# nizepart/Research-and-Development-of-Kubernetes-Operator-for-Machine-Learning-Pipelines

Hardware: AMD Instinct MI355X
Metric: served_tokens_per_sec (higher is better)
Workload: dtype bf16

## Files before the change

### research-and-development-of-kubernetes-operator-for-machine-learning-pipelines_amd/ops/csrc/bindings.cpp

```cpp
#include <cstdlib>
#include <string>
#include <torch/library.h>
#include <ATen/ATen.h>
#include <c10/hip/HIPStream.h>
#include <c10/core/DeviceGuard.h>
#include <cmath>

#include "launch.h"
#include "gemm_plan.h"

namespace {

using at::Tensor;

hipStream_t cur_stream() { return c10::hip::getCurrentHIPStream().stream(); }

void check_bf16(const Tensor& t, const char* name) {
  TORCH_CHECK(t.is_cuda(), name, " must be a GPU tensor");
  TORCH_CHECK(t.scalar_type() == at::kBFloat16, name, " must be bf16");
  TORCH_CHECK(t.is_contiguous(), name, " must be contiguous");
}
void check_i32(const Tensor& t, const char* name) {
  TORCH_CHECK(t.is_cuda(), name, " must be a GPU tensor");
  TORCH_CHECK(t.scalar_type() == at::kInt, name, " must be int32");
// ... 898 lines not shown
  const long H = mlop::ep_hidden((long)h), k = mlop::ep_topk((long)h);
  check_bf16(out, "out"); check_bf16(y, "y"); check_i32(topi, "topi");
  TORCH_CHECK(topw.scalar_type() == at::kFloat && topw.is_cuda() && topw.is_contiguous(), "topw fp32");
  TORCH_CHECK(out.dim() == 2 && out.size(1) == H && y.dim() == 2 && y.size(1) == H, "ep_combine: [*, H] rows");
  TORCH_CHECK(topw.numel() == out.size(0) * k && topi.numel() == out.size(0) * k, "ep_combine: [T, k] routing");
  c10::DeviceGuard g(out.device());
  mlop::ep_combine((long)h, out.data_ptr(), y.data_ptr(), (long)y.size(0), topw.data_ptr<float>(),
                   topi.data_ptr<int>(), (int)out.size(0), cur_stream());
}
int64_t ep_error(int64_t h) { return mlop::ep_error((long)h); }
int64_t ep_mem_mode(int64_t h) { return mlop::ep_mem_mode((long)h); }
void ep_destroy(int64_t h) { mlop::ep_destroy((long)h); }

}

extern "C" const char* mlop_src_hash();
std::string src_hash() { return std::string(mlop_src_hash()); }

TORCH_LIBRARY(mlop, m) {
  m.def("src_hash() -> str", &src_hash);
  m.def("device_delay(int us) -> ()", &device_delay);
  m.def("car_create(int rank, int world, int max_bytes, int device, bool split=False) -> int", &car_create);
  m.def("car_ipc_handle(int h) -> Tensor", &car_ipc_handle);
  m.def("car_open(int h, Tensor handles) -> ()", &car_open);
  m.def("car_all_reduce(int h, Tensor(a!) out, Tensor inp, bool two_shot=False) -> ()");
  m.def("car_all_reduce_add(int h, Tensor(a!) residual, Tensor inp) -> ()");
  m.def("car_broadcast(int h, Tensor(a!) buf, int root) -> ()");
  m.def("car_all_gather(int h, Tensor(a!) out, Tensor piece) -> ()");
  m.def("car_error(int h) -> int", &car_error);
  m.def("attn_fused_max_pairs(int n) -> int", &attn_fused_max_pairs);
  m.def("car_mem_mode(int h) -> int", &car_mem_mode);
  m.def("car_destroy(int h) -> ()", &car_destroy);
  m.def("chan_create(str name, int slots, int consumers) -> int", &chan_create);
  m.def("chan_open(str name) -> int", &chan_open);
  m.def("chan_send(int h, Tensor vals, int timeout_us) -> bool", &chan_send);
  m.def("chan_recv(int h, int consumer, Tensor(a!) out, int timeout_us) -> bool", &chan_recv);
  m.def("chan_unlink(str name) -> ()", &chan_unlink);
  m.def("chan_close(int h, bool unlink) -> ()", &chan_close);
  m.def("xg_create(str name, int world, int slots, int max_words) -> int", &xg_create);
  m.def("xg_open(str name, int rank) -> int", &xg_open);
  m.def("xg_exchange(int h, Tensor vals, Tensor(a!) out, Tensor(b!) counts, int timeout_us) -> bool", &xg_exchange);
  m.def("xg_close(int h) -> ()", &xg_close);
  m.def("ep_create(int rank, int world, int E, int k, int H, int tcap, int device) -> int", &ep_create);
  m.def("ep_ipc_handle(int h) -> Tensor", &ep_ipc_handle);
  m.def("ep_open(int h, Tensor handles) -> ()", &ep_open);
  m.def("ep_dispatch(int h, Tensor(a!) xp, Tensor(b!) offsets, Tensor x, Tensor topi) -> ()");
  m.def("ep_combine(int h, Tensor(a!) out, Tensor y, Tensor topw, Tensor topi) -> ()");
  m.def("ep_error(int h) -> int", &ep_error);
  m.def("ep_mem_mode(int h) -> int", &ep_mem_mode);
  m.def("ep_destroy(int h) -> ()", &ep_destroy);
  m.def("gemm_workspace(int M, int N, int K, int epi) -> int", &gemm_workspace);
  m.def("gemm_big_variant(int set=-1) -> int", &knob<mlop::gemm_big_variant>);
  m.def("gemm_half_tile(int set=-1) -> int", &knob<mlop::gemm_half_tile>);
  m.def("gemm_small_nt(int set=-1) -> int", &knob<mlop::gemm_small_nt>);
  m.def("attn_kv_nt(int set=-1) -> int", &knob<mlop::attn_kv_nt>);
  m.def("gemm_slab_nt(int set=-1) -> int", &knob<mlop::gemm_slab_nt>);
  m.def("gemm_rope_split(int set=-1) -> int", &knob<mlop::gemm_rope_split>);
  m.def("gemm_split_target(int set=-1) -> int", &knob<mlop::gemm_split_target>);
  m.def("gemm_grouped_narrow(int set=-1) -> int", &knob<mlop::gemm_grouped_narrow>);
  m.def("gemm_ws_max_m(int set=-1) -> int", &knob<mlop::gemm_ws_max_m>);
  m.def("decode_chain_max_m() -> int", &decode_chain_max_m);
  m.def("gemm_ws_plan(int rb, int u, int nt) -> ()", &gemm_ws_plan);
  m.def("gemm_ws_small_m(int set=-1) -> int", &knob<mlop::gemm_ws_small_m>);
  m.def("gemm_ws_rope_m(int set=-1) -> int", &knob<mlop::gemm_ws_rope_m>);
  m.def("flash_persist(int set=-1) -> int", &knob<mlop::flash_persist>);
  m.def("flash_stream(int set=-1) -> int", &knob<mlop::flash_stream>);
  m.def("gemm_grouped_balance(int set=-1) -> int", &knob<mlop::gemm_grouped_balance>);
  m.def("gemm_grouped_order(int set=-1) -> int", &knob<mlop::gemm_grouped_order>);
  m.def("moe_mid_tok(int set=-1) -> int", &knob<mlop::moe_mid_tok>);
  m.def("gemm_mid_chain(int set=-1) -> int", &knob<mlop::gemm_mid_chain>);
  m.def("mid_chain_ok(int M, int N, int K, int epi) -> bool", &mid_chain_ok);
  m.def("moe_mid_max_tokens(int set=-1) -> int", &knob<mlop::moe_mid_max_tokens>);
  m.def("gemm_grouped_plan(int bm, int bn, int stages, int splits) -> ()", &gemm_grouped_plan);
  m.def("gemm_dense_plan(int variant, int bm, int bn, int splits, int stages=0) -> ()", &gemm_dense_plan);
  m.def("gemm_small_stages(int set=-1) -> int", &knob<mlop::gemm_small_stages>);
  m.def("gemm_small_tile(int set=-1) -> int", &knob<mlop::gemm_small_tile>);
  m.def("gemm_sk_mode(int set=-1) -> int", &knob<mlop::gemm_sk_mode>);
  m.def("gemm_sk_reserve() -> bool", &gemm_sk_reserve);
  m.def("gemm_sk_workgroups(int M, int N, int K) -> int", &gemm_sk_workgroups);
  m.def("vmm_supported(int device) -> bool", &vmm_supported);
  m.def("vmm_granularity(int device) -> int", &vmm_granularity);
  m.def("vmm_arena(int bytes, int device) -> Tensor", &vmm_arena);
  m.def("vmm_map_chunks(Tensor flat, int region_stride, int n_regions, int chunk_bytes, int first, "
        "int count, bool async_) -> bool", &vmm_map_chunks);
  m.def("vmm_chunks_ready(Tensor flat) -> int", &vmm_chunks_ready);
  m.def("vmm_error(Tensor flat) -> int", &vmm_error);
  m.def("gemm_rope_supported(int M, int N, int K) -> bool", &gemm_rope_supported);
  m.def("w4_chain_ok(int M, int N, int K) -> bool", &w4_chain_ok);
  m.def("chain_ok(int M, int N, int K, int epi) -> bool", &chain_ok);
  m.def("gemm_route(int M, int N, int K, int op, int n_groups=0, int rows_per_group=0) -> int[]", &gemm_route);
  m.def("gemm_route_env(int M, int N, int K, int op, int cus, bool sk, int n_groups=0, int rows_per_group=0) -> int[]", &gemm_route_env);
  m.def("gemm_tile_configs() -> int[]", &gemm_tile_configs);
  m.def("gemm_res_ss(Tensor(a!) residual, Tensor a, Tensor w, Tensor(b!) ss_out) -> bool");
  m.def("gemm_rs(Tensor(a!) out, Tensor a, Tensor w, Tensor ss_in, float eps, int epi) -> bool");
  m.def("gemm_rs_rope(Tensor(a!) q_out, Tensor(b!) k_cache, Tensor(c!) v_cache, Tensor a, Tensor w, "
        "Tensor pos, Tensor cos_sin, Tensor slots, Tensor ss_in, float eps) -> bool");
  m.def("gemm_rope_cache(Tensor(a!) q_out, Tensor(b!) k_cache, Tensor(c!) v_cache, Tensor a, Tensor w, "
        "Tensor pos, Tensor cos_sin, Tensor slots) -> bool");
  m.def("gemm(Tensor(a!) out, Tensor a, Tensor w, Tensor(b!) ws, int epi) -> ()");
  m.def("grouped_gemm(Tensor(a!) out, Tensor a, Tensor w, Tensor offsets, int max_rows, "
        "int epi, Tensor? a_rows=None) -> ()");
  m.def("gemm_add_rmsnorm(Tensor(a!) out, Tensor(b!) residual, Tensor a, Tensor w, Tensor norm_w, "
        "Tensor(c!) ws, float eps) -> bool");
  m.def("gemv_chain_supported(int M, int N, int K, int epi) -> bool", &gemv_chain_supported);
  m.def("moe_route(Tensor(a!) topw, Tensor(b!) topi, Tensor logits) -> ()");
  m.def("moe_permute(Tensor(a!) xp, Tensor(b!) offsets, Tensor(c!) src, Tensor(d!) inv, Tensor x, "
// ... 86 lines not shown
```

### research-and-development-of-kubernetes-operator-for-machine-learning-pipelines_amd/ops/csrc/gemm_plan.cc

```cpp
#include "gemm_plan.h"

#include <algorithm>
#include <stddef.h>
#include <stdexcept>

namespace mlop {

namespace {
enum { EPI_NONE = 0, EPI_SILU_MUL = 1, EPI_ROPE = 3 };
enum { WS_NONE = 0, WS_SILU_MUL = 1, WS_ROPE = 3, WS_RES = 5 };
constexpr int kHeadD = 128;
constexpr int kGroupedSmallStages = 3;
}

static PlanEnv g_knobs;
PlanEnv& gemm_knobs() { return g_knobs; }

int gemm_split_target(int set) {
  if (set >= 1) g_knobs.split_target = set;
  return g_knobs.split_target;
}

int gemm_small_stages(int set) {
  if (set >= 0) g_knobs.small_stages = set;
  return g_knobs.small_stages;
}

int gemm_small_tile(int set) {
  if (set >= 0) g_knobs.small_tile = set;
  return g_knobs.small_tile;
}

static bool tile_shape_built(int bm, int bn, bool grouped) {
  for (const TileCfg& t : kGemmTiles)
    if (t.BM == bm && t.BN == bn && (grouped || !(bm == 256 && bn == 256))) return true;
  return false;
}

void gemm_grouped_plan(int bm, int bn, int stages, int splits) {
  if (bm > 0 && !tile_shape_built(bm, bn, true))
    throw std::runtime_error("gemm_grouped_plan: no grouped config for this tile");
  int* gp = g_knobs.gp;
  gp[0] = bm, gp[1] = bn, gp[2] = stages, gp[3] = splits;
}

void gemm_dense_plan(int variant, int bm, int bn, int splits, int stages) {
  if (variant >= 0 && variant != 0 && variant != 1 && variant != 3 && variant != 5 && variant != 6)
    throw std::runtime_error("gemm_dense_plan: variant must be 0, 1, 3, 5 or 6");
  if (variant == 0 && !tile_shape_built(bm, bn, false))
    throw std::runtime_error("gemm_dense_plan: no dense config for this tile");
  int* dp = g_knobs.dp;
  dp[0] = variant, dp[1] = bm, dp[2] = bn, dp[3] = splits, dp[4] = stages > 0 ? stages : 0;
}

int gemm_big_variant(int set) {
  if (set >= 0) g_knobs.big_variant = set;
  return g_knobs.big_variant;
}
int gemm_grouped_narrow(int set) {
  if (set >= 0) g_knobs.grouped_narrow = set;
  return g_knobs.grouped_narrow;
}
int gemm_half_tile(int set) {
  if (set >= 0) g_knobs.half_tile = set;
  return g_knobs.half_tile;
}

int gemm_sk_mode(int set) {
  if (set >= 0) g_knobs.sk_mode = set;
  return g_knobs.sk_mode;
}

int gemm_rope_split(int set) {
  if (set >= 1) g_knobs.rope_split_k = set;
  return g_knobs.rope_split_k;
}

int gemm_mid_chain(int set) {
  if (set >= 0) g_knobs.mid_chain = set;
  return g_knobs.mid_chain;
}

int gemm_ws_max_m(int set) {
  if (set >= 0) g_knobs.ws_max_m = set > 64 ? 64 : set;
  return g_knobs.ws_max_m;
}

int gemm_ws_small_m(int set) {
  if (set >= 0) g_knobs.ws_small_m = set > 64 ? 64 : set;
  return g_knobs.ws_small_m;
}

int gemm_ws_rope_m(int set) {
  if (set >= 0) g_knobs.ws_rope_m = set > 64 ? 64 : set;
  return g_knobs.ws_rope_m;
}


bool gemv_takes(const PlanEnv& e, int M, int N, int K, int epi) {
  if (M < 1 || M > e.gemv_max_m || K % 8 || N < 4) return false;
  if (epi == EPI_SILU_MUL) return N % 32 == 0;
  if (epi == EPI_ROPE) return N % kHeadD == 0;
  return epi == EPI_NONE && N % 4 == 0;
}

bool gemv_grouped_takes(int M, int N, int K, int epi) {
  return M >= 1 && M <= 8 && K % 8 == 0 && N % (epi == EPI_SILU_MUL ? 32 : 4) == 0 &&
         (epi == EPI_NONE || epi == EPI_SILU_MUL);
}

bool gemv_chain_takes(const PlanEnv& e, int M, int N, int K, int epi) {
  return M <= e.gemv_chain_max_m && gemv_takes(e, M, N, K, epi);
}

bool ws_prefer(const PlanEnv& e, int M, int N, int K, int epi) {
  if (M <= e.gemv_chain_max_m || (long)N * K > 32L * 1024 * 1024 || K % 512) return false;
  if (epi == WS_ROPE) return M <= e.ws_rope_m && N % 128 == 0;
  return M <= e.ws_small_m && (epi == WS_NONE || epi == WS_RES) && N % 16 == 0;
// ... 407 lines not shown
```

### research-and-development-of-kubernetes-operator-for-machine-learning-pipelines_amd/ops/csrc/gemm_plan.h

```cpp
#pragma once

#if defined(__HIP__) || defined(__HIPCC__)
#define MLOP_HD __host__ __device__
#else
#define MLOP_HD
#endif

namespace mlop {

constexpr int kBK = 64;
constexpr int kMaxSplits = 8;
constexpr int kSkMaxWg = 256;
constexpr long kSkScratchFloats = 2l * kSkMaxWg * 256 * 256;
constexpr int kSkMinIters = 16;
constexpr int sk_min_half() { return kSkMinIters / 2 > 1 ? kSkMinIters / 2 : 1; }

MLOP_HD inline int sk_choose_d(int T, int nk, int cus, int min_half) {
  const int r = T % cus;
  if (r == 0) return 0;
  float best = 0.9f * nk;
  int best_d = 0;
  const int dmax = cus / r < 32 ? cus / r : 32;
  for (int d = 2; d <= dmax; ++d) {
    if (nk % d || nk / d < min_half) continue;
    const float w = 0.04f * r * d;
    const float cost = nk / d + (w > 2.f ? w : 2.f) + 2.f * (d >= 3 ? d : d - 1) + 1.f;
    if (cost < best) {
      best = cost;
      best_d = d;
    }
  }
  return best_d;
}

struct PlanEnv {
  int cus = 0;
  bool sk = false;
  int small_tile = 1;
  int small_stages = 3;
  int big_variant = 5;
  int half_tile = 1;
  int grouped_narrow = 1;
  int split_target = 512;
  int rope_split_k = 2;
  int sk_mode = 1;
  int mid_chain = 0;
  int gp[4] = {-1, -1, -1, -1};
  int dp[5] = {-1, -1, -1, -1, 0};
  int ws_small_m = 8, ws_rope_m = 8, ws_max_m = 0;
  int gemv_max_m = 4, gemv_chain_max_m = 4;
  bool sk_on() const { return sk_mode && sk && cus > 0; }
};
PlanEnv& gemm_knobs();
PlanEnv gemm_live_env();
int gemm_small_tile(int set);
int gemm_small_stages(int set);
int gemm_big_variant(int set);
int gemm_half_tile(int set);
int gemm_grouped_narrow(int set);
int gemm_split_target(int set);
int gemm_rope_split(int set);
int gemm_sk_mode(int set);
int gemm_mid_chain(int set);
int gemm_ws_small_m(int set);
int gemm_ws_rope_m(int set);
int gemm_ws_max_m(int set);

enum GemmOp {
  OP_PLAIN = 0,
  OP_SILU_MUL = 1,
  OP_ADD_RMSNORM = 2,
  OP_ROPE = 3,
  OP_CHAIN_RES_SS = 4,
  OP_CHAIN_RS = 8,
  OP_CHAIN_RS_SILU = 9,
  OP_CHAIN_RS_ROPE = 11,
  OP_GROUPED = 16,
  OP_GROUPED_SILU = 17,
};

struct GemmCall {
  int op = OP_PLAIN;
  int M = 0, N = 0, K = 0;
  int lda = 0, ldb = 0, ldc = 0;
  int n_groups = 0, rows_per_group = 0;
  long ws_avail = -1;
  bool indirect = false;
};

enum GemmFamily { FAM_REFUSED = 0, FAM_GEMV, FAM_WS, FAM_TILE, FAM_PP, FAM_W4, FAM_W4H };
enum GemmFinish { FIN_NONE = 0, FIN_REDUCE, FIN_ADD_RMSNORM, FIN_ROPE_SLABS, FIN_RMSNORM };
enum GemmWsSrc { WS_SRC_NONE = 0, WS_SRC_CALLER, WS_SRC_SCRATCH };

#define MLOP_GEMM_TILES(X)       \
  X(16, 32, 1, 2, 8, false, 0)   \
  X(16, 32, 1, 2, 6, false, 0)   \
  X(16, 32, 1, 2, 4, false, 0)   \
  X(16, 64, 1, 2, 8, false, 0)   \
  X(16, 64, 1, 2, 6, false, 0)   \
  X(16, 64, 1, 2, 4, false, 0)   \
  X(32, 32, 1, 2, 8, false, 0)   \
  X(32, 32, 1, 2, 4, false, 0)   \
  X(32, 64, 1, 4, 6, false, 0)   \
  X(32, 64, 1, 4, 4, false, 0)   \
  X(64, 32, 1, 2, 4, false, 0)   \
  X(64, 64, 1, 4, 6, false, 0)   \
  X(64, 64, 1, 4, 4, false, 0)   \
  X(64, 64, 1, 4, 3, false, 0)   \
  X(128, 64, 2, 2, 5, false, 0)  \
  X(128, 64, 2, 2, 3, false, 0)  \
  X(256, 64, 4, 2, 3, false, 0)  \
// ... 52 lines not shown
```

### research-and-development-of-kubernetes-operator-for-machine-learning-pipelines_amd/ops/csrc/gemm_w4.hip

```cpp
#include "common.h"
#include "launch.h"
#include "gemm_plan.h"
#include "gemm_w4_asm.h"

#include <type_traits>
#include <utility>

namespace mlop {

namespace {
enum { W4_NONE = 0, W4_SILU_MUL = 1, W4_ROPE = 3, W4_ADD_SS = 4, W4_RS = 8 };
using i32x4 = __attribute__((ext_vector_type(4))) int;
typedef __attribute__((address_space(3))) uint16_t lds_u16;

__device__ __forceinline__ i32x4 make_srd(const void* p) {
  const uint64_t a = (uint64_t)p;
  i32x4 r;
  r.x = __builtin_amdgcn_readfirstlane((int)(uint32_t)a);
  r.y = __builtin_amdgcn_readfirstlane((int)(uint32_t)(a >> 32));
  r.z = 0x7fffffff;
  r.w = 0x00020000;
  return r;
}

template <int I>
__device__ __forceinline__ void read_block(float (&v)[32]) {
#define MLOP_W4_OUTS                                                                                   \
  "=v"(v[0]), "=v"(v[1]), "=v"(v[2]), "=v"(v[3]), "=v"(v[4]), "=v"(v[5]), "=v"(v[6]), "=v"(v[7]),     \
      "=v"(v[8]), "=v"(v[9]), "=v"(v[10]), "=v"(v[11]), "=v"(v[12]), "=v"(v[13]), "=v"(v[14]),         \
      "=v"(v[15]), "=v"(v[16]), "=v"(v[17]), "=v"(v[18]), "=v"(v[19]), "=v"(v[20]), "=v"(v[21]),       \
      "=v"(v[22]), "=v"(v[23]), "=v"(v[24]), "=v"(v[25]), "=v"(v[26]), "=v"(v[27]), "=v"(v[28]),       \
      "=v"(v[29]), "=v"(v[30]), "=v"(v[31])
  if constexpr (I == 0) asm volatile(MLOP_W4_READ0_ASM : MLOP_W4_OUTS);
  else if constexpr (I == 1) asm volatile(MLOP_W4_READ1_ASM : MLOP_W4_OUTS);
  else if constexpr (I == 2) asm volatile(MLOP_W4_READ2_ASM : MLOP_W4_OUTS);
  else if constexpr (I == 3) asm volatile(MLOP_W4_READ3_ASM : MLOP_W4_OUTS);
  else if constexpr (I == 4) asm volatile(MLOP_W4_READ4_ASM : MLOP_W4_OUTS);
  else if constexpr (I == 5) asm volatile(MLOP_W4_READ5_ASM : MLOP_W4_OUTS);
  else if constexpr (I == 6) asm volatile(MLOP_W4_READ6_ASM : MLOP_W4_OUTS);
  else asm volatile(MLOP_W4_READ7_ASM : MLOP_W4_OUTS);
#undef MLOP_W4_OUTS
}

template <typename F, int... I>
__device__ __forceinline__ void unroll_impl(F& f, std::integer_sequence<int, I...>) {
  (f(std::integral_constant<int, I>{}), ...);
}
template <int N, typename F>
__device__ __forceinline__ void unroll(F&& f) {
  unroll_impl(f, std::make_integer_sequence<int, N>{});
}
}

template <int EPI, int BMT>
__global__ void __launch_bounds__(256, 1) gemm_w4_kernel(
    const uint16_t* __restrict__ A, int lda, const uint16_t* __restrict__ B, int ldb,
    uint16_t* __restrict__ C, int ldc, int M, int N, int K, int n_tiles_x, int m_tiles, int group_m,
    RopeEpi re, int n_dp, int n_items, float* __restrict__ ws, int* __restrict__ cnt) {
  constexpr int BM = BMT, BN = 256;
  static_assert(BMT == 256 || BMT == 128, "tile heights of the generated K-loops");
  constexpr int NI = BMT / 32;
  constexpr int NPC = NI + 8;
  constexpr int BASE = EPI & 3;
  constexpr bool ADD = (EPI & W4_ADD_SS) != 0, RS = (EPI & W4_RS) != 0;
  static_assert(!ADD || BASE == W4_NONE, "residual add on the plain epilogue only");
  constexpr int NS = BASE == W4_SILU_MUL ? 2 * NI : 4 * NI;
  extern __shared__ __attribute__((aligned(16))) uint16_t smem[];
  const int tid = threadIdx.x, lane = tid & 63;
  const int wid = __builtin_amdgcn_readfirstlane(tid >> 6);
  const int wm = wid >> 1, wn = wid & 1;
  const int nk = K / 64;

  const int G = gridDim.x, Lb = blockIdx.x;
  const int q = G >> 3, rr = G & 7, xcd = Lb & 7, slot = Lb >> 3;
  const int lid = (xcd < rr ? xcd * (q + 1) : rr * (q + 1) + (xcd - rr) * q) + slot;
  auto origin = [&](int t, int& m0, int& n0) {
    const int band = t / (group_m * n_tiles_x), in_band = t % (group_m * n_tiles_x);
    const int gm_here = min(group_m, m_tiles - band * group_m);
    m0 = (band * group_m + in_band % gm_here) * BM;
    n0 = (in_band / gm_here) * BN;
    if constexpr (BASE == W4_ROPE) n0 = (n_tiles_x - 1) * BN - n0;
  };
  auto item = [&](int i, int& m0, int& n0, int& kb, int& nkl) {
    const bool tail = i >= n_dp;
    origin(tail ? n_dp + ((i - n_dp) >> 1) : i, m0, n0);
    kb = tail ? ((i - n_dp) & 1) * (nk >> 1) : 0;
    nkl = tail ? nk >> 1 : nk;
  };
  auto dma_offsets = [&](int m0, int n0, int kb, uint32_t (&vo)[NPC]) {
#pragma unroll
    for (int i = 0; i < NPC; ++i) {
      const int p = wid + 4 * i;
      const int r = (i < NI ? p : p - 4 * NI) * 8 + (lane >> 3);
      const uint32_t ch = (uint32_t)(((lane & 7) ^ ((r >> 1) & 7)) << 4);
      if (i < NI) vo[i] = (uint32_t)min(m0 + r, M - 1) * (uint32_t)(lda * 2) + ch + kb * 128;
      else vo[i] = (uint32_t)min(n0 + r, N - 1) * (uint32_t)(ldb * 2) + ch + kb * 128;
    }
  };
  const i32x4 srdA = make_srd(A), srdB = make_srd(B);
  const auto srdC = __builtin_amdgcn_make_buffer_rsrc((void*)C, 0, (int)((uint32_t)M * (uint32_t)ldc * 2u), 0x00020000);
  const uint32_t lbase = (uint32_t)(uintptr_t)((lds_u16*)smem);
  const uint32_t sw = ((lane & 15) >> 1) & 7;
  const uint32_t c0 = (((uint32_t)(lane >> 4)) ^ sw) << 4, c1 = (((uint32_t)(lane >> 4) + 4) ^ sw) << 4;
  const uint32_t a_row = lbase + (uint32_t)(wm * (BMT / 2) + (lane & 15)) * 128;
  const uint32_t b_row = lbase + BMT * 128 + (uint32_t)(wn * 128 + (lane & 15)) * 128;
  const uint32_t dbase0 = __builtin_amdgcn_readfirstlane(lbase + wid * 1024);
  const uint32_t k128 = 128;
  float* rinv_lds = reinterpret_cast<float*>(smem + 65536);
  int* band_flag = reinterpret_cast<int*>(smem + 65536 + 1024);

  for (int it = lid, first = 1; it < n_items; it += G, first = 0) {
    int m0, n0, kb, nkl;
    item(it, m0, n0, kb, nkl);
    uint32_t vo[NPC], vn[NPC];
    dma_offsets(m0, n0, kb, vo);
    const bool next = it + G < n_items;
    {
      int m1 = m0, n1 = n0, kb1 = kb, nkl1 = nkl;
      if (next) item(it + G, m1, n1, kb1, nkl1);
      dma_offsets(m1, n1, kb1, vn);
    }
    if constexpr (RS) {
      const auto rs_ss = __builtin_amdgcn_make_buffer_rsrc((void*)re.ss_in, 0, (int)((uint32_t)M * 4u), 0x00020000);
      const uint32_t voff = (uint32_t)(m0 + wm * (BMT / 2) + lane) * 4u;
      const uint32_t lds_dst = __builtin_amdgcn_readfirstlane(lbase + 131072u + (uint32_t)wid * 512u);
      uint32_t msave;
      asm volatile(
          "s_mov_b32 %[ms], m0\n"
          "s_mov_b32 m0, %[dst]\n"
          "s_nop 0\n"
          "buffer_load_dword %[vo], %[srd], 0 offen lds\n"
          "s_add_u32 m0, m0, 0x100\n"
          "s_nop 0\n"
          "buffer_load_dword %[vo2], %[srd], 0 offen lds\n"
          "s_mov_b32 m0, %[ms]\n"
          : [ms] "=&s"(msave)
          : [dst] "s"(lds_dst), [vo] "v"(voff), [vo2] "v"(voff + 256u), [srd] "s"(rs_ss)
          : "memory", "scc");
    }
    uint32_t rA0 = a_row + c0, rA1 = a_row + c1, rB0 = b_row + c0, rB1 = b_row + c1;
    uint32_t dbase = dbase0, koff = 256, m0save;
    uint32_t iter = __builtin_amdgcn_readfirstlane(nkl - 3);
    const uint32_t s_first = __builtin_amdgcn_readfirstlane(first), s_next = __builtin_amdgcn_readfirstlane((int)next);
    bf16x8 fa0_0, fa0_1, fa0_2, fa0_3, fa0_4, fa0_5, fa0_6, fa0_7;
    bf16x8 fb0_0, fb0_1, fb0_2, fb0_3, fb0_4, fb0_5, fb0_6, fb0_7;
    bf16x8 fa1_0, fa1_1, fa1_2, fa1_3, fa1_4, fa1_5, fa1_6, fa1_7;
    bf16x8 fb1_0, fb1_1, fb1_2, fb1_3, fb1_4, fb1_5, fb1_6, fb1_7;
#define MLOP_W4_OPERANDS                                                                                         \
  : [fa0_0] "=&v"(fa0_0), [fa0_1] "=&v"(fa0_1), [fa0_2] "=&v"(fa0_2), [fa0_3] "=&v"(fa0_3),                      \
    [fa0_4] "=&v"(fa0_4), [fa0_5] "=&v"(fa0_5), [fa0_6] "=&v"(fa0_6), [fa0_7] "=&v"(fa0_7),                      \
    [fb0_0] "=&v"(fb0_0), [fb0_1] "=&v"(fb0_1), [fb0_2] "=&v"(fb0_2), [fb0_3] "=&v"(fb0_3),                      \
    [fb0_4] "=&v"(fb0_4), [fb0_5] "=&v"(fb0_5), [fb0_6] "=&v"(fb0_6), [fb0_7] "=&v"(fb0_7),                      \
    [fa1_0] "=&v"(fa1_0), [fa1_1] "=&v"(fa1_1), [fa1_2] "=&v"(fa1_2), [fa1_3] "=&v"(fa1_3),                      \
    [fa1_4] "=&v"(fa1_4), [fa1_5] "=&v"(fa1_5), [fa1_6] "=&v"(fa1_6), [fa1_7] "=&v"(fa1_7),                      \
    [fb1_0] "=&v"(fb1_0), [fb1_1] "=&v"(fb1_1), [fb1_2] "=&v"(fb1_2), [fb1_3] "=&v"(fb1_3),                      \
    [fb1_4] "=&v"(fb1_4), [fb1_5] "=&v"(fb1_5), [fb1_6] "=&v"(fb1_6), [fb1_7] "=&v"(fb1_7),                      \
    [rA0] "+v"(rA0), [rA1] "+v"(rA1), [rB0] "+v"(rB0), [rB1] "+v"(rB1), [koff] "+s"(koff), [dbase] "+s"(dbase), \
    [iter] "+s"(iter), [m0save] "=&s"(m0save)                                                                    \
  : [vo0] "v"(vo[0]), [vo1] "v"(vo[1]), [vo2] "v"(vo[2]), [vo3] "v"(vo[3]), [vo4] "v"(vo[4]), [vo5] "v"(vo[5]), \
    [vo6] "v"(vo[6]), [vo7] "v"(vo[7]), [vo8] "v"(vo[8]), [vo9] "v"(vo[9]), [vo10] "v"(vo[10]),                 \
    [vo11] "v"(vo[11]), [vo12] "v"(vo[12]), [vo13] "v"(vo[13]), [vo14] "v"(vo[14]), [vo15] "v"(vo[15]),         \
    [vn0] "v"(vn[0]), [vn1] "v"(vn[1]), [vn2] "v"(vn[2]), [vn3] "v"(vn[3]), [vn4] "v"(vn[4]), [vn5] "v"(vn[5]), \
    [vn6] "v"(vn[6]), [vn7] "v"(vn[7]), [vn8] "v"(vn[8]), [vn9] "v"(vn[9]), [vn10] "v"(vn[10]),                 \
    [vn11] "v"(vn[11]), [vn12] "v"(vn[12]), [vn13] "v"(vn[13]), [vn14] "v"(vn[14]), [vn15] "v"(vn[15]),         \
    [srdA] "s"(srdA), [srdB] "s"(srdB), [k128] "s"(k128), [first] "s"(s_first), [has_next] "s"(s_next)          \
  : "memory", "scc", MLOP_W4_AGPR_CLOBBERS
#define MLOP_W4H_OPERANDS                                                                                        \
  : [fa0_0] "=&v"(fa0_0), [fa0_1] "=&v"(fa0_1), [fa0_2] "=&v"(fa0_2), [fa0_3] "=&v"(fa0_3),                      \
    [fb0_0] "=&v"(fb0_0), [fb0_1] "=&v"(fb0_1), [fb0_2] "=&v"(fb0_2), [fb0_3] "=&v"(fb0_3),                      \
    [fb0_4] "=&v"(fb0_4), [fb0_5] "=&v"(fb0_5), [fb0_6] "=&v"(fb0_6), [fb0_7] "=&v"(fb0_7),                      \
    [fa1_0] "=&v"(fa1_0), [fa1_1] "=&v"(fa1_1), [fa1_2] "=&v"(fa1_2), [fa1_3] "=&v"(fa1_3),                      \
    [fb1_0] "=&v"(fb1_0), [fb1_1] "=&v"(fb1_1), [fb1_2] "=&v"(fb1_2), [fb1_3] "=&v"(fb1_3),                      \
    [fb1_4] "=&v"(fb1_4), [fb1_5] "=&v"(fb1_5), [fb1_6] "=&v"(fb1_6), [fb1_7] "=&v"(fb1_7),                      \
    [rA0] "+v"(rA0), [rA1] "+v"(rA1), [rB0] "+v"(rB0), [rB1] "+v"(rB1), [koff] "+s"(koff), [dbase] "+s"(dbase), \
    [iter] "+s"(iter), [m0save] "=&s"(m0save)                                                                    \
  : [vo0] "v"(vo[0]), [vo1] "v"(vo[1]), [vo2] "v"(vo[2]), [vo3] "v"(vo[3]), [vo4] "v"(vo[4]), [vo5] "v"(vo[5]), \
    [vo6] "v"(vo[6]), [vo7] "v"(vo[7]), [vo8] "v"(vo[8]), [vo9] "v"(vo[9]), [vo10] "v"(vo[10]),                 \
    [vo11] "v"(vo[11]), [vn0] "v"(vn[0]), [vn1] "v"(vn[1]), [vn2] "v"(vn[2]), [vn3] "v"(vn[3]),                 \
    [vn4] "v"(vn[4]), [vn5] "v"(vn[5]), [vn6] "v"(vn[6]), [vn7] "v"(vn[7]), [vn8] "v"(vn[8]), [vn9] "v"(vn[9]), \
    [vn10] "v"(vn[10]), [vn11] "v"(vn[11]), [srdA] "s"(srdA), [srdB] "s"(srdB), [k128] "s"(k128),               \
    [first] "s"(s_first), [has_next] "s"(s_next)                                                                 \
  : "memory", "scc", MLOP_W4_AGPR_CLOBBERS
    constexpr int NQ = NS + (RS ? 2 : 0);
    if constexpr (BMT == 256) {
      static_assert(NQ == 32 || NQ == 16 || NQ == 34 || NQ == 18, "one generated K-loop per VMEM count");
      if constexpr (NQ == 32) asm volatile(MLOP_W4_KLOOP_S32_P0_ASM MLOP_W4_OPERANDS);
      else if constexpr (NQ == 16) asm volatile(MLOP_W4_KLOOP_S16_P0_ASM MLOP_W4_OPERANDS);
      else if constexpr (NQ == 34) asm volatile(MLOP_W4_KLOOP_S34_P0_ASM MLOP_W4_OPERANDS);
      else asm volatile(MLOP_W4_KLOOP_S18_P0_ASM MLOP_W4_OPERANDS);
    } else {
      static_assert(NQ == 16 || NQ == 8 || NQ == 18 || NQ == 10, "one generated K-loop per VMEM count");
      if constexpr (NQ == 16) asm volatile(MLOP_W4H_KLOOP_S16_ASM MLOP_W4H_OPERANDS);
      else if constexpr (NQ == 8) asm volatile(MLOP_W4H_KLOOP_S8_ASM MLOP_W4H_OPERANDS);
      else if constexpr (NQ == 18) asm volatile(MLOP_W4H_KLOOP_S18_ASM MLOP_W4H_OPERANDS);
      else asm volatile(MLOP_W4H_KLOOP_S10_ASM MLOP_W4H_OPERANDS);
    }
#undef MLOP_W4_OPERANDS
#undef MLOP_W4H_OPERANDS

    const int lr = wm * (BMT / 2) + (lane & 15), qd = lane >> 4;
    const bool part = it >= n_dp;
    const int sidx = part ? it - n_dp : 0;
    const auto rs_other = __builtin_amdgcn_make_buffer_rsrc(part ? ws + (size_t)(sidx ^ 1) * 65536 : (float*)C, 0,
                                                           65536 * 4, 0x00020000);
    if (part) {
      const int tt = sidx >> 1;
      const auto rs_own = __builtin_amdgcn_make_buffer_rsrc(ws + (size_t)sidx * 65536, 0, 65536 * 4, 0x00020000);
      auto put = [&](auto I_) {
        constexpr int I = decltype(I_)::value;
        float v[32];
        read_block<I>(v);
#pragma unroll
        for (int q4 = 0; q4 < 8; ++q4)
          __builtin_amdgcn_raw_buffer_store_b128(
              u32x4{__float_as_uint(v[4 * q4]), __float_as_uint(v[4 * q4 + 1]), __float_as_uint(v[4 * q4 + 2]),
                    __float_as_uint(v[4 * q4 + 3])},
              rs_own, (uint32_t)(((I * 8 + q4) * 256 + tid) * 16), 0, 16 );
      };
      unroll<NI>(put);
      asm volatile("s_waitcnt vmcnt(0)" ::: "memory");
      __syncthreads();
      int* flag = reinterpret_cast<int*>(smem);
      if (tid == 0) {
        const int tk = __hip_atomic_fetch_add(cnt + tt, 1, __ATOMIC_RELAXED, __HIP_MEMORY_SCOPE_AGENT);
        if (tk == 1) __hip_atomic_store(cnt + tt, 0, __ATOMIC_RELAXED, __HIP_MEMORY_SCOPE_AGENT);
        flag[0] = tk == 1;
      }
      __syncthreads();
      const int last = flag[0];
      __syncthreads();
      if (!last) break;
    }
    auto fetch = [&](auto I_, float (&v)[32]) {
      constexpr int I = decltype(I_)::value;
      read_block<I>(v);
      if (part) {
#pragma unroll
        for (int b4 = 0; b4 < 8; b4 += 4) {
          u32x4 o[4];
#pragma unroll
          for (int q4 = 0; q4 < 4; ++q4)
            o[q4] = __builtin_bit_cast(u32x4, __builtin_amdgcn_raw_buffer_load_b128(
                                                  rs_other, (uint32_t)(((I * 8 + b4 + q4) * 256 + tid) * 16), 0, 16 ));
#pragma unroll
          for (int q4 = 0; q4 < 4; ++q4)
#pragma unroll
            for (int e = 0; e < 4; ++e) v[4 * (b4 + q4) + e] += __uint_as_float(o[q4][e]);
        }
      }
      if constexpr (RS) {
        const float f = rsqrtf(rinv_lds[wid * 128 + 16 * I + (lane & 15)] * re.ss_inv_k + re.ss_eps);
#pragma unroll
        for (int e = 0; e < 32; ++e) v[e] *= f;
      }
    };
    const int odd = qd & 1, half = qd >> 1;
    auto swap_f = [&](const float* x, const float* y, float (&lo)[4], float (&hi)[4]) {
#pragma unroll
      for (int r = 0; r < 4; ++r) {
        const auto sw2 = __builtin_amdgcn_permlane16_swap(__float_as_uint(x[r]), __float_as_uint(y[r]), false, false);
        lo[r] = __uint_as_float(sw2[0]);
        hi[r] = __uint_as_float(sw2[1]);
      }
    };
    auto swap_pair = [&](const float* x, const float* y, u32x4& out) {
      float lo[4], hi[4];
      swap_f(x, y, lo, hi);
      out = u32x4{pack2(lo[0], lo[1]), pack2(lo[2], lo[3]), pack2(hi[0], hi[1]), pack2(hi[2], hi[3])};
    };
    if constexpr (BASE == W4_ROPE) {
      constexpr int D = 128, HALF = 64;
      const bool r_nt = (re.ws_nt & 8) != 0;
      auto put16 = [&](uint16_t* p, const u32x4& v) {
        if (r_nt) __builtin_nontemporal_store(v, reinterpret_cast<u32x4*>(p));
        else *reinterpret_cast<u32x4*>(p) = v;
      };
      const int head = (n0 + wn * 128) / D;
      const int n_rope = re.Hq + re.Hkv, n_all = re.Hq + 2 * re.Hkv;
      if (head >= n_all) {
      } else if (head >= n_rope) {
        const int kh = head - n_rope;
        int sl[NI];
#pragma unroll
        for (int I = 0; I < NI; ++I) {
          const int m = m0 + lr + I * 16;
          sl[I] = m < M ? re.slots[m] : -1;
        }
        auto vstore = [&](auto I_) {
          constexpr int I = decltype(I_)::value;
          float v[32];
          fetch(I_, v);
          u32x4 d[4];
#pragma unroll
          for (int pr = 0; pr < 4; ++pr) swap_pair(v + 8 * pr, v + 8 * pr + 4, d[pr]);
          const int slot = sl[I];
          if (slot < 0) return;
          uint16_t* dst = re.v_cache + (((size_t)(slot / re.BS) * re.Hkv + kh) * re.BS + slot % re.BS) * D;
#pragma unroll
          for (int pr = 0; pr < 4; ++pr)
            put16(dst + (2 * pr + odd) * 16 + 8 * half, d[pr]);
        };
        unroll<NI>(vstore);
      } else {
        const bool is_k = head >= re.Hq;
        int pp[NI], sl[NI];
#pragma unroll
        for (int I = 0; I < NI; ++I) {
          const int m = m0 + lr + I * 16;
          const bool ok = m < M;
          pp[I] = ok ? re.pos[m] : 0;
          sl[I] = ok && is_k ? re.slots[m] : -1;
        }
        const int c0 = 4 * qd;
        auto load_cs = [&](int I, float4 (&cs)[8]) {
          const float4* cr = reinterpret_cast<const float4*>(re.cos_sin + (size_t)pp[I] * D);
#pragma unroll
          for (int j = 0; j < 4; ++j) {
            cs[j] = cr[(j * 16 + c0) / 4];
            cs[4 + j] = cr[(HALF + j * 16 + c0) / 4];
          }
        };
        auto rstore = [&](auto I_, const float4 (&cs)[8], float4 (&nxt)[8]) {
          constexpr int I = decltype(I_)::value;
          if constexpr (I < NI - 1) load_cs(I + 1, nxt);
          float v[32];
          fetch(I_, v);
          float xo[4][4], yo[4][4];
#pragma unroll
          for (int j = 0; j < 4; ++j) {
            const float cv[4] = {cs[j].x, cs[j].y, cs[j].z, cs[j].w};
            const float sv[4] = {cs[4 + j].x, cs[4 + j].y, cs[4 + j].z, cs[4 + j].w};
#pragma unroll
            for (int r = 0; r < 4; ++r) {
              const float x = bf2f(f2bf(v[4 * j + r])), y = bf2f(f2bf(v[4 * (j + 4) + r]));
              xo[j][r] = x * cv[r] - y * sv[r];
              yo[j][r] = y * cv[r] + x * sv[r];
            }
          }
          u32x4 d[4];
          swap_pair(xo[0], xo[1], d[0]);
          swap_pair(xo[2], xo[3], d[1]);
          swap_pair(yo[0], yo[1], d[2]);
          swap_pair(yo[2], yo[3], d[3]);
          const int m = m0 + lr + I * 16;
          if (m >= M) return;
          uint16_t* dst;
          if (!is_k) {
            dst = re.q_out + ((size_t)m * re.Hq + head) * D;
          } else {
            const int slot = sl[I];
            if (slot < 0) return;
            dst = re.k_cache + (((size_t)(slot / re.BS) * re.Hkv + (head - re.Hq)) * re.BS + slot % re.BS) * D;
          }
#pragma unroll
          for (int b = 0; b < 4; ++b)
            put16(dst + (b >> 1) * HALF + ((b & 1) * 2 + odd) * 16 + 8 * half, d[b]);
        };
        float4 csa[8], csb[8];
        load_cs(0, csa);
        unroll<NI>([&](auto I_) {
          if constexpr (decltype(I_)::value % 2 == 0) rstore(I_, csa, csb);
          else rstore(I_, csb, csa);
        });
      }
    } else {
      const int col_w = BASE == W4_NONE ? n0 + wn * 128 : (n0 + wn * 128) / 2;
      const bool c_nt = (re.ws_nt & 2) != 0;
      const int n_groups = N >> 7, g_out = (n0 + wn * 128) >> 7;
      const auto rs_sso = __builtin_amdgcn_make_buffer_rsrc((void*)re.ss_out, 0, ADD ? (int)((uint32_t)M * n_groups * 4u) : 0,
                                                            0x00020000);
      auto store = [&](auto I_) {
        constexpr int I = decltype(I_)::value;
        float v[32];
        fetch(I_, v);
        const uint32_t row_off = (uint32_t)(m0 + lr + I * 16) * (uint32_t)ldc * 2u;
        if constexpr (BASE == W4_SILU_MUL) {
          float o[16];
#pragma unroll
          for (int jp = 0; jp < 4; ++jp)
#pragma unroll
            for (int r = 0; r < 4; ++r) o[4 * jp + r] = silu_bf(v[8 * jp + r]) * bf2f(f2bf(v[8 * jp + 4 + r]));
#pragma unroll
          for (int pr = 0; pr < 2; ++pr) {
            u32x4 d;
            swap_pair(o + 8 * pr, o + 8 * pr + 4, d);
            const int col = col_w + (2 * pr + odd) * 16 + 8 * half;
            if (c_nt) __builtin_amdgcn_raw_buffer_store_b128(d, srdC, row_off + col * 2, 0, 2 );
            else __builtin_amdgcn_raw_buffer_store_b128(d, srdC, row_off + col * 2, 0, 0);
          }
// ... 37 lines not shown
          for (int e = 0; e < 8; ++e) ssq += h[e] * h[e];
          const int col = col_w + (2 * pr + odd) * 16 + 8 * half;
          const u32x4 hv{pack2(h[0], h[1]), pack2(h[2], h[3]), pack2(h[4], h[5]), pack2(h[6], h[7])};
          if (c_nt) __builtin_amdgcn_raw_buffer_store_b128(hv, srdC, row_off + col * 2, 0, 2 );
          else __builtin_amdgcn_raw_buffer_store_b128(hv, srdC, row_off + col * 2, 0, 0);
        }
        ssq += __shfl_xor(ssq, 16);
        ssq += __shfl_xor(ssq, 32);
        if (qd == 0)
          __builtin_amdgcn_raw_buffer_store_b32(__float_as_uint(ssq), rs_sso,
                                                ((uint32_t)(m0 + lr + I * 16) * n_groups + g_out) * 4u, 0, 16 );
      };
      if constexpr (ADD) {
        u32x4 ra[4], rb[4];
        load_res(0, ra);
        unroll<NI>([&](auto I_) {
          if constexpr (decltype(I_)::value % 2 == 0) store_add(I_, ra, rb);
          else store_add(I_, rb, ra);
        });
      } else {
        unroll<NI>(store);
      }
      if constexpr (ADD) {
        asm volatile("s_waitcnt vmcnt(0)" ::: "memory");
        __syncthreads();
        const int band = m0 / BM;
        if (tid == 0) {
          const int tk = __hip_atomic_fetch_add(re.ss_cnt + band, 1, __ATOMIC_RELAXED, __HIP_MEMORY_SCOPE_AGENT);
          const int lastb = tk == n_tiles_x - 1;
          if (lastb) __hip_atomic_store(re.ss_cnt + band, 0, __ATOMIC_RELAXED, __HIP_MEMORY_SCOPE_AGENT);
          band_flag[0] = lastb;
        }
        __syncthreads();
        if (band_flag[0]) {
          const int r = m0 + tid;
          if (tid < BM && r < M) {
            float sum = 0.f;
            int c = 0;
            for (; c + 4 <= n_groups; c += 4) {
              const u32x4 x = __builtin_bit_cast(
                  u32x4, __builtin_amdgcn_raw_buffer_load_b128(rs_sso, (uint32_t)(r * n_groups + c) * 4u, 0, 16 ));
              sum += __uint_as_float(x[0]) + __uint_as_float(x[1]) + __uint_as_float(x[2]) + __uint_as_float(x[3]);
            }
            if (c < n_groups) {
              const u32x2 x = __builtin_bit_cast(
                  u32x2, __builtin_amdgcn_raw_buffer_load_b64(rs_sso, (uint32_t)(r * n_groups + c) * 4u, 0, 16 ));
              sum += __uint_as_float(x[0]) + __uint_as_float(x[1]);
            }
            re.ss_tot[r] = sum;
          }
        }
      }
    }
  }
}

template <int EPI, int BMT>
static bool run_w4_t(const uint16_t* A, int lda, const uint16_t* B, int ldb, uint16_t* C, int ldc, int M, int N,
                     int K, hipStream_t st, const RopeEpi& re) {
  constexpr size_t ring = 2ull * 65536 + ((EPI & (W4_RS | W4_ADD_SS)) ? 4 * 128 * 4 + 16 : 0);
  constexpr size_t stg = 0;
  constexpr size_t lds = ring > stg ? ring : stg;
  static_assert(lds <= 163840, "LDS budget");
  auto kern = gemm_w4_kernel<EPI, BMT>;
  static bool attr = false;
  if (!attr) {
    (void)hipFuncSetAttribute((const void*)kern, hipFuncAttributeMaxDynamicSharedMemorySize, (int)lds);
    attr = true;
  }
  const int gx = (N + 255) / 256, gy = (M + BMT - 1) / BMT;
  constexpr int group_m = 1024 / BMT;
  const int gm = std::max(1, std::min(group_m, gy));
  const int T = gx * gy;
  int n_dp = T, n_items = T;
  float* ws = nullptr;
  int* cnt = nullptr;
  int cus = 256;
  if (gemm_w4_split_ok(gemm_live_env(), T, K / 64)) {
    int c2 = 0;
    if (gemm_sk_scratch(&ws, &cnt, &c2)) {
      n_dp = T - T % c2;
      n_items = n_dp + 2 * (T % c2);
    }
  }
  int grid = n_items;
  if (!gemm_sk_available(&cus) || cus <= 0) {
    static int cu_count[16] = {};
    int dev = 0;
    (void)hipGetDevice(&dev);
    if (dev >= 0 && dev < 16 && cu_count[dev] == 0)
      (void)hipDeviceGetAttribute(&cu_count[dev], hipDeviceAttributeMultiprocessorCount, dev);
    cus = (dev >= 0 && dev < 16 && cu_count[dev] > 0) ? cu_count[dev] : 256;
  }
  grid = std::min(grid, cus);
  RopeEpi re2 = re;
  re2.ws_nt = gemm_slab_nt(-1);
  if constexpr ((EPI & W4_ADD_SS) != 0) {
    float* w2 = nullptr;
    int c3 = 0;
    if (!gemm_sk_scratch(&w2, &re2.ss_cnt, &c3)) return false;
  }
  kern<<<grid, 256, lds, st>>>(A, lda, B, ldb, C, ldc, M, N, K, gx, gy, gm, re2, n_dp, n_items, ws, cnt);
  return true;
}

template <int BMT>
static bool run_w4_h(int epi, const uint16_t* A, int lda, const uint16_t* B, int ldb, uint16_t* C, int ldc, int M,
                     int N, int K, hipStream_t st, const RopeEpi& re) {
  switch (epi) {
    case W4_NONE: return run_w4_t<W4_NONE, BMT>(A, lda, B, ldb, C, ldc, M, N, K, st, re);
    case W4_SILU_MUL: return run_w4_t<W4_SILU_MUL, BMT>(A, lda, B, ldb, C, ldc, M, N, K, st, re);
    case W4_ROPE: return run_w4_t<W4_ROPE, BMT>(A, lda, B, ldb, C, ldc, M, N, K, st, re);
    case W4_ADD_SS: return run_w4_t<W4_ADD_SS, BMT>(A, lda, B, ldb, C, ldc, M, N, K, st, re);
    case W4_NONE | W4_RS: return run_w4_t<W4_NONE | W4_RS, BMT>(A, lda, B, ldb, C, ldc, M, N, K, st, re);
    case W4_SILU_MUL | W4_RS: return run_w4_t<W4_SILU_MUL | W4_RS, BMT>(A, lda, B, ldb, C, ldc, M, N, K, st, re);
    case W4_ROPE | W4_RS: return run_w4_t<W4_ROPE | W4_RS, BMT>(A, lda, B, ldb, C, ldc, M, N, K, st, re);
    default: return false;
  }
}

bool run_w4(int epi, const uint16_t* A, int lda, const uint16_t* B, int ldb, uint16_t* C, int ldc, int M, int N,
            int K, hipStream_t st, const RopeEpi& re, int bm) {
  if (bm == 128) return run_w4_h<128>(epi, A, lda, B, ldb, C, ldc, M, N, K, st, re);
  if (bm == 256) return run_w4_h<256>(epi, A, lda, B, ldb, C, ldc, M, N, K, st, re);
  return false;
}

}
```

Baseline: 37880.

## Split W4 GEMM tail tiles into half-height row items to balance CUs

Adds a second way to handle the partial last wave of the persistent W4 GEMM. Leftover tiles are split into two 128-row halves, each run by a separate workgroup with a BM=128 instantiation of the K-loop, instead of only splitting along K. Row splitting needs no scratch reduction or cross-workgroup flag sync. Tail planning moves into a shared host/device helper, a knob is added, and the RoPE math now uses FMA with constant-offset buffer stores. The cost is a larger kernel with two inlined item bodies, which may raise register pressure.

New measurement: 38190 (median of 6 runs). Within noise of the previous version (+0.8%).

```diff
diff --git a/research-and-development-of-kubernetes-operator-for-machine-learning-pipelines_amd/ops/csrc/bindings.cpp b/research-and-development-of-kubernetes-operator-for-machine-learning-pipelines_amd/ops/csrc/bindings.cpp
--- a/research-and-development-of-kubernetes-operator-for-machine-learning-pipelines_amd/ops/csrc/bindings.cpp
+++ b/research-and-development-of-kubernetes-operator-for-machine-learning-pipelines_amd/ops/csrc/bindings.cpp
@@ -974,6 +974,7 @@
   m.def("gemm_workspace(int M, int N, int K, int epi) -> int", &gemm_workspace);
   m.def("gemm_big_variant(int set=-1) -> int", &knob<mlop::gemm_big_variant>);
   m.def("gemm_half_tile(int set=-1) -> int", &knob<mlop::gemm_half_tile>);
+  m.def("gemm_w4_tail(int set=-1) -> int", &knob<mlop::gemm_w4_tail>);
   m.def("gemm_small_nt(int set=-1) -> int", &knob<mlop::gemm_small_nt>);
   m.def("attn_kv_nt(int set=-1) -> int", &knob<mlop::attn_kv_nt>);
   m.def("gemm_slab_nt(int set=-1) -> int", &knob<mlop::gemm_slab_nt>);
diff --git a/research-and-development-of-kubernetes-operator-for-machine-learning-pipelines_amd/ops/csrc/gemm_plan.cc b/research-and-development-of-kubernetes-operator-for-machine-learning-pipelines_amd/ops/csrc/gemm_plan.cc
--- a/research-and-development-of-kubernetes-operator-for-machine-learning-pipelines_amd/ops/csrc/gemm_plan.cc
+++ b/research-and-development-of-kubernetes-operator-for-machine-learning-pipelines_amd/ops/csrc/gemm_plan.cc
@@ -64,6 +64,11 @@
 int gemm_half_tile(int set) {
   if (set >= 0) g_knobs.half_tile = set;
   return g_knobs.half_tile;
+}
+
+int gemm_w4_tail(int set) {
+  if (set >= 0) g_knobs.w4_tail = set;
+  return g_knobs.w4_tail;
 }
 
 int gemm_sk_mode(int set) {
diff --git a/research-and-development-of-kubernetes-operator-for-machine-learning-pipelines_amd/ops/csrc/gemm_plan.h b/research-and-development-of-kubernetes-operator-for-machine-learning-pipelines_amd/ops/csrc/gemm_plan.h
--- a/research-and-development-of-kubernetes-operator-for-machine-learning-pipelines_amd/ops/csrc/gemm_plan.h
+++ b/research-and-development-of-kubernetes-operator-for-machine-learning-pipelines_amd/ops/csrc/gemm_plan.h
@@ -33,6 +33,35 @@
   return best_d;
 }
 
+enum W4Tail { W4_TAIL_NONE = 0, W4_TAIL_K = 1, W4_TAIL_ROWS = 2 };
+enum { W4_CAP_K = 1, W4_CAP_ROWS = 2 };
+struct W4Items {
+  int n_dp, n_tail, kind;
+  MLOP_HD int n_items() const { return n_dp + 2 * n_tail; }
+};
+MLOP_HD inline W4Items w4_items(int T, int cus, int nk, int epi, int caps) {
+  W4Items it{T, 0, W4_TAIL_NONE};
+  if (T <= 0 || cus <= 0) return it;
+  const int r = T % cus, n_dp = T - r;
+  if (r == 0 || 2 * r > cus) return it;
+  if ((caps & W4_CAP_ROWS) && n_dp > 0 && !(epi & 4)) return W4Items{n_dp, r, W4_TAIL_ROWS};
+  if ((caps & W4_CAP_K) && nk % 2 == 0 && nk / 2 >= 3) return W4Items{n_dp, r, W4_TAIL_K};
+  return it;
+}
+struct W4Item {
+  int tile, h, kb, nkl, row0;
+};
+MLOP_HD inline W4Item w4_item(const W4Items& s, int i, int nk) {
+  if (i < s.n_dp || s.kind == W4_TAIL_NONE) return W4Item{i, 0, 0, nk, 0};
+  const int j = (i - s.n_dp) >> 1, h = (i - s.n_dp) & 1;
+  if (s.kind == W4_TAIL_K) return W4Item{s.n_dp + j, h, h * (nk >> 1), nk >> 1, 0};
+  return W4Item{s.n_dp + j, h, 0, nk, 128 * h};
+}
+MLOP_HD inline int w4_lid(int G, int b) {
+  const int q = G >> 3, rr = G & 7, xcd = b & 7, slot = b >> 3;
+  return (xcd < rr ? xcd * (q + 1) : rr * (q + 1) + (xcd - rr) * q) + slot;
+}
+
 struct PlanEnv {
   int cus = 0;
   bool sk = false;
@@ -40,6 +69,7 @@
   int small_stages = 3;
   int big_variant = 5;
   int half_tile = 1;
+  int w4_tail = 1;
   int grouped_narrow = 1;
   int split_target = 512;
   int rope_split_k = 2;
@@ -57,6 +87,7 @@
 int gemm_small_stages(int set);
 int gemm_big_variant(int set);
 int gemm_half_tile(int set);
+int gemm_w4_tail(int set);
 int gemm_grouped_narrow(int set);
 int gemm_split_target(int set);
 int gemm_rope_split(int set);
diff --git a/research-and-development-of-kubernetes-operator-for-machine-learning-pipelines_amd/ops/csrc/gemm_w4.hip b/research-and-development-of-kubernetes-operator-for-machine-learning-pipelines_amd/ops/csrc/gemm_w4.hip
--- a/research-and-development-of-kubernetes-operator-for-machine-learning-pipelines_amd/ops/csrc/gemm_w4.hip
+++ b/research-and-development-of-kubernetes-operator-for-machine-learning-pipelines_amd/ops/csrc/gemm_w4.hip
@@ -56,24 +56,22 @@
 __global__ void __launch_bounds__(256, 1) gemm_w4_kernel(
     const uint16_t* __restrict__ A, int lda, const uint16_t* __restrict__ B, int ldb,
     uint16_t* __restrict__ C, int ldc, int M, int N, int K, int n_tiles_x, int m_tiles, int group_m,
-    RopeEpi re, int n_dp, int n_items, float* __restrict__ ws, int* __restrict__ cnt) {
+    RopeEpi re, int cus, int caps, float* __restrict__ ws, int* __restrict__ cnt) {
   constexpr int BM = BMT, BN = 256;
   static_assert(BMT == 256 || BMT == 128, "tile heights of the generated K-loops");
-  constexpr int NI = BMT / 32;
-  constexpr int NPC = NI + 8;
   constexpr int BASE = EPI & 3;
   constexpr bool ADD = (EPI & W4_ADD_SS) != 0, RS = (EPI & W4_RS) != 0;
   static_assert(!ADD || BASE == W4_NONE, "residual add on the plain epilogue only");
-  constexpr int NS = BASE == W4_SILU_MUL ? 2 * NI : 4 * NI;
   extern __shared__ __attribute__((aligned(16))) uint16_t smem[];
   const int tid = threadIdx.x, lane = tid & 63;
   const int wid = __builtin_amdgcn_readfirstlane(tid >> 6);
   const int wm = wid >> 1, wn = wid & 1;
   const int nk = K / 64;
 
-  const int G = gridDim.x, Lb = blockIdx.x;
-  const int q = G >> 3, rr = G & 7, xcd = Lb & 7, slot = Lb >> 3;
-  const int lid = (xcd < rr ? xcd * (q + 1) : rr * (q + 1) + (xcd - rr) * q) + slot;
+  const W4Items items = w4_items(n_tiles_x * m_tiles, cus, nk, EPI, caps);
+  const int n_dp = items.n_dp, n_items = items.n_items();
+  const int G = gridDim.x;
+  const int lid = w4_lid(G, blockIdx.x);
   auto origin = [&](int t, int& m0, int& n0) {
     const int band = t / (group_m * n_tiles_x), in_band = t % (group_m * n_tiles_x);
     const int gm_here = min(group_m, m_tiles - band * group_m);
@@ -82,39 +80,47 @@
     if constexpr (BASE == W4_ROPE) n0 = (n_tiles_x - 1) * BN - n0;
   };
   auto item = [&](int i, int& m0, int& n0, int& kb, int& nkl) {
-    const bool tail = i >= n_dp;
-    origin(tail ? n_dp + ((i - n_dp) >> 1) : i, m0, n0);
-    kb = tail ? ((i - n_dp) & 1) * (nk >> 1) : 0;
-    nkl = tail ? nk >> 1 : nk;
-  };
-  auto dma_offsets = [&](int m0, int n0, int kb, uint32_t (&vo)[NPC]) {
-#pragma unroll
-    for (int i = 0; i < NPC; ++i) {
-      const int p = wid + 4 * i;
-      const int r = (i < NI ? p : p - 4 * NI) * 8 + (lane >> 3);
-      const uint32_t ch = (uint32_t)(((lane & 7) ^ ((r >> 1) & 7)) << 4);
-      if (i < NI) vo[i] = (uint32_t)min(m0 + r, M - 1) * (uint32_t)(lda * 2) + ch + kb * 128;
-      else vo[i] = (uint32_t)min(n0 + r, N - 1) * (uint32_t)(ldb * 2) + ch + kb * 128;
-    }
+    const W4Item w = w4_item(items, i, nk);
+    origin(w.tile, m0, n0);
+    m0 += w.row0;
+    kb = w.kb;
+    nkl = w.nkl;
   };
   const i32x4 srdA = make_srd(A), srdB = make_srd(B);
   const auto srdC = __builtin_amdgcn_make_buffer_rsrc((void*)C, 0, (int)((uint32_t)M * (uint32_t)ldc * 2u), 0x00020000);
   const uint32_t lbase = (uint32_t)(uintptr_t)((lds_u16*)smem);
   const uint32_t sw = ((lane & 15) >> 1) & 7;
   const uint32_t c0 = (((uint32_t)(lane >> 4)) ^ sw) << 4, c1 = (((uint32_t)(lane >> 4) + 4) ^ sw) << 4;
-  const uint32_t a_row = lbase + (uint32_t)(wm * (BMT / 2) + (lane & 15)) * 128;
-  const uint32_t b_row = lbase + BMT * 128 + (uint32_t)(wn * 128 + (lane & 15)) * 128;
+  const uint32_t lrow = lbase + (uint32_t)(lane & 15) * 128;
   const uint32_t dbase0 = __builtin_amdgcn_readfirstlane(lbase + wid * 1024);
   const uint32_t k128 = 128;
   float* rinv_lds = reinterpret_cast<float*>(smem + 65536);
   int* band_flag = reinterpret_cast<int*>(smem + 65536 + 1024);
 
-  for (int it = lid, first = 1; it < n_items; it += G, first = 0) {
+  auto run_item = [&](auto H_, auto KH_, const int it, const int first, const bool next) __attribute__((always_inline)) -> bool {
+    constexpr int H = decltype(H_)::value;
+    constexpr bool KH = decltype(KH_)::value;
+    constexpr int NI = H / 32;
+    constexpr int NPC = NI + 8;
+    constexpr int NS = BASE == W4_SILU_MUL ? 2 * NI : 4 * NI;
+    uint32_t lrow_i = lrow;
+    asm volatile("" : "+v"(lrow_i));
+    const uint32_t a_row = lrow_i + (uint32_t)(wm * (H / 2)) * 128;
+    const uint32_t b_row = lrow_i + H * 128 + (uint32_t)(wn * 128) * 128;
+    auto dma_offsets = [&](int m0, int n0, int kb, uint32_t (&vo)[NPC]) {
+#pragma unroll
+      for (int i = 0; i < NPC; ++i) {
+        const int p = wid + 4 * i;
+        const int r = (i < NI ? p : p - 4 * NI) * 8 + (lane >> 3);
+        const uint32_t ch = (uint32_t)(((lane & 7) ^ ((r >> 1) & 7)) << 4);
+        if (i < NI) vo[i] = (uint32_t)min(m0 + r, M - 1) * (uint32_t)(lda * 2) + ch + kb * 128;
+        else vo[i] = (uint32_t)min(n0 + r, N - 1) * (uint32_t)(ldb * 2) + ch + kb * 128;
+      }
+    };
     int m0, n0, kb, nkl;
     item(it, m0, n0, kb, nkl);
     uint32_t vo[NPC], vn[NPC];
     dma_offsets(m0, n0, kb, vo);
-    const bool next = it + G < n_items;
     {
       int m1 = m0, n1 = n0, kb1 = kb, nkl1 = nkl;
       if (next) item(it + G, m1, n1, kb1, nkl1);
@@ -122,7 +128,7 @@
     }
     if constexpr (RS) {
       const auto rs_ss = __builtin_amdgcn_make_buffer_rsrc((void*)re.ss_in, 0, (int)((uint32_t)M * 4u), 0x00020000);
-      const uint32_t voff = (uint32_t)(m0 + wm * (BMT / 2) + lane) * 4u;
+      const uint32_t voff = (uint32_t)(m0 + wm * (H / 2) + lane) * 4u;
       const uint32_t lds_dst = __builtin_amdgcn_readfirstlane(lbase + 131072u + (uint32_t)wid * 512u);
       uint32_t msave;
       asm volatile(
@@ -182,7 +188,7 @@
     [first] "s"(s_first), [has_next] "s"(s_next)                                                                 \
   : "memory", "scc", MLOP_W4_AGPR_CLOBBERS
     constexpr int NQ = NS + (RS ? 2 : 0);
-    if constexpr (BMT == 256) {
+    if constexpr (H == 256) {
       static_assert(NQ == 32 || NQ == 16 || NQ == 34 || NQ == 18, "one generated K-loop per VMEM count");
       if constexpr (NQ == 32) asm volatile(MLOP_W4_KLOOP_S32_P0_ASM MLOP_W4_OPERANDS);
       else if constexpr (NQ == 16) asm volatile(MLOP_W4_KLOOP_S16_P0_ASM MLOP_W4_OPERANDS);
@@ -198,8 +204,8 @@
 #undef MLOP_W4_OPERANDS
 #undef MLOP_W4H_OPERANDS
 
-    const int lr = wm * (BMT / 2) + (lane & 15), qd = lane >> 4;
-    const bool part = it >= n_dp;
+    const int lr = wm * (H / 2) + (lane & 15), qd = lane >> 4;
+    const bool part = KH && items.kind == W4_TAIL_K && it >= n_dp;
     const int sidx = part ? it - n_dp : 0;
     const auto rs_other = __builtin_amdgcn_make_buffer_rsrc(part ? ws + (size_t)(sidx ^ 1) * 65536 : (float*)C, 0,
                                                            65536 * 4, 0x00020000);
@@ -210,12 +216,14 @@
         constexpr int I = decltype(I_)::value;
         float v[32];
         read_block<I>(v);
+        uint32_t so = I * 8 * 4096;
+        asm volatile("" : "+s"(so));
 #pragma unroll
         for (int q4 = 0; q4 < 8; ++q4)
           __builtin_amdgcn_raw_buffer_store_b128(
               u32x4{__float_as_uint(v[4 * q4]), __float_as_uint(v[4 * q4 + 1]), __float_as_uint(v[4 * q4 + 2]),
                     __float_as_uint(v[4 * q4 + 3])},
-              rs_own, (uint32_t)(((I * 8 + q4) * 256 + tid) * 16), 0, 16 );
+              rs_own, (uint32_t)tid * 16u, so + q4 * 4096, 16 );
       };
       unroll<NI>(put);
       asm volatile("s_waitcnt vmcnt(0)" ::: "memory");
@@ -229,19 +237,21 @@
       __syncthreads();
       const int last = flag[0];
       __syncthreads();
-      if (!last) break;
+      if (!last) return false;
     }
     auto fetch = [&](auto I_, float (&v)[32]) {
       constexpr int I = decltype(I_)::value;
       read_block<I>(v);
       if (part) {
+        uint32_t so = I * 8 * 4096;
+        asm volatile("" : "+s"(so));
 #pragma unroll
         for (int b4 = 0; b4 < 8; b4 += 4) {
           u32x4 o[4];
 #pragma unroll
           for (int q4 = 0; q4 < 4; ++q4)
             o[q4] = __builtin_bit_cast(u32x4, __builtin_amdgcn_raw_buffer_load_b128(
-                                                  rs_other, (uint32_t)(((I * 8 + b4 + q4) * 256 + tid) * 16), 0, 16 ));
+                                                  rs_other, (uint32_t)tid * 16u, so + (b4 + q4) * 4096, 16 ));
 #pragma unroll
           for (int q4 = 0; q4 < 4; ++q4)
 #pragma unroll
@@ -333,8 +343,8 @@
 #pragma unroll
             for (int r = 0; r < 4; ++r) {
               const float x = bf2f(f2bf(v[4 * j + r])), y = bf2f(f2bf(v[4 * (j + 4) + r]));
-              xo[j][r] = x * cv[r] - y * sv[r];
-              yo[j][r] = y * cv[r] + x * sv[r];
+              xo[j][r] = __builtin_fmaf(x, cv[r], -(y * sv[r]));
+              yo[j][r] = __builtin_fmaf(y, cv[r], x * sv[r]);
             }
           }
           u32x4 d[4];
@@ -478,6 +488,19 @@
         }
       }
     }
+    return true;
+  };
+
+  using std::integral_constant;
+  for (int it = lid, first = 1; it < n_items; it += G, first = 0) {
+    if constexpr (BMT == 256 && !ADD) {
+      if (items.kind == W4_TAIL_ROWS && it >= n_dp) {
+        run_item(integral_constant<int, 128>{}, integral_constant<bool, false>{}, it, 1, false);
+        break;
+      }
+    }
+    const bool next = it + G < n_items && !(items.kind == W4_TAIL_ROWS && it + G >= n_dp);
+    if (!run_item(integral_constant<int, BMT>{}, integral_constant<bool, true>{}, it, first, next)) break;
   }
 }
 
@@ -498,19 +521,12 @@
   constexpr int group_m = 1024 / BMT;
   const int gm = std::max(1, std::min(group_m, gy));
   const int T = gx * gy;
-  int n_dp = T, n_items = T;
   float* ws = nullptr;
   int* cnt = nullptr;
   int cus = 256;
-  if (gemm_w4_split_ok(gemm_live_env(), T, K / 64)) {
-    int c2 = 0;
-    if (gemm_sk_scratch(&ws, &cnt, &c2)) {
-      n_dp = T - T % c2;
-      n_items = n_dp + 2 * (T % c2);
-    }
-  }
-  int grid = n_items;
-  if (!gemm_sk_available(&cus) || cus <= 0) {
+  const PlanEnv env = gemm_live_env();
+  const bool sk = env.sk_on() && gemm_sk_available(&cus) && cus > 0;
+  if (!sk) {
     static int cu_count[16] = {};
     int dev = 0;
     (void)hipGetDevice(&dev);
@@ -518,7 +534,16 @@
       (void)hipDeviceGetAttribute(&cu_count[dev], hipDeviceAttributeMultiprocessorCount, dev);
     cus = (dev >= 0 && dev < 16 && cu_count[dev] > 0) ? cu_count[dev] : 256;
   }
-  grid = std::min(grid, cus);
+  int caps = (sk ? W4_CAP_K : 0) | (BMT == 256 && env.w4_tail ? W4_CAP_ROWS : 0);
+  W4Items items = w4_items(T, cus, K / 64, EPI, caps);
+  if (items.kind == W4_TAIL_K) {
+    int c2 = 0;
+    if (!gemm_sk_scratch(&ws, &cnt, &c2) || c2 != cus) {
+      caps &= ~W4_CAP_K;
+      items = w4_items(T, cus, K / 64, EPI, caps);
+    }
+  }
+  const int grid = std::min(items.n_items(), cus);
   RopeEpi re2 = re;
   re2.ws_nt = gemm_slab_nt(-1);
   if constexpr ((EPI & W4_ADD_SS) != 0) {
@@ -526,7 +551,7 @@
     int c3 = 0;
     if (!gemm_sk_scratch(&w2, &re2.ss_cnt, &c3)) return false;
   }
-  kern<<<grid, 256, lds, st>>>(A, lda, B, ldb, C, ldc, M, N, K, gx, gy, gm, re2, n_dp, n_items, ws, cnt);
+  kern<<<grid, 256, lds, st>>>(A, lda, B, ldb, C, ldc, M, N, K, gx, gy, gm, re2, cus, caps, ws, cnt);
   return true;
 }
 
```
